# jwwangchn/BONAI

Measured on AMD Instinct MI355X. Metric: training img/s at 1024x1024 LOFT R50-FPN, higher is better.
Workload: dtype bf16; 1 GPU; LOFT R50-FPN + FOA, 8x1024x1024 synthetic tiles per GPU (BASELINE configs[1]), 80 gt/img, full train step (fwd+losses+bwd+allreduce+clip+SGD), random-init weights, RoI heads at the load of a trained RPN (first proposals = jittered gt boxes); global_batch=8, per_gpu_batch=8, parallelism=dp1, graph_features=False

## Files before the change

bonai_amd/csrc/elementwise.hip:

```cpp
#include "loft_common.h"
#include "../../include/loft_hip.h"
#include "conv_tap.h"

__device__ __forceinline__ void ld8(const bf16_t* p, float v[8]) {
    uint4 t = *reinterpret_cast<const uint4*>(p);
    unpack8_16(t, v);
}
__device__ __forceinline__ void st8(bf16_t* p, const float v[8]) {
    *reinterpret_cast<uint4*>(p) = pack8_16(v);
}

__device__ __forceinline__ void ld8(const float* p, float v[8]) { ld4(p, v); ld4(p + 4, v + 4); }
__device__ __forceinline__ void st8(float* p, const float v[8]) { st4(p, v); st4(p + 4, v + 4); }

static inline dim3 ew_grid(long nvec) {
    long b = (nvec + 255) / 256;
    if (b > 8192) b = 8192;
    if (b < 1) b = 1;
    return dim3((unsigned)b);
}

__global__ void relu_bwd_kernel(const bf16_t* __restrict__ g, const bf16_t* __restrict__ y, bf16_t* __restrict__ out,
                                long nvec) {
    for (long i = blockIdx.x * (long)blockDim.x + threadIdx.x; i < nvec; i += (long)gridDim.x * blockDim.x) {
// ... 1140 lines not shown
        const int r = i >> 5, cp = (i & 31) * 2;
        uint32_t v = 0;
        if (r0 + r < R && c0 + cp < Cc) v = *reinterpret_cast<const uint32_t*>(src + (long)(r0 + r) * Cc + c0 + cp);
        t[r][cp] = (bf16_t)(v & 0xffff);
        t[r][cp + 1] = (bf16_t)(v >> 16);
    }
    __syncthreads();
    for (int i = threadIdx.x; i < 64 * 32; i += 256) {
        const int c = i >> 5, rp = (i & 31) * 2;
        if (c0 + c < Cc && r0 + rp < R)
            *reinterpret_cast<uint32_t*>(dst + (long)(c0 + c) * R + r0 + rp) = (uint32_t)t[rp][c] | ((uint32_t)t[rp + 1][c] << 16);
    }
}
LOFT_EXPORT int loft_transpose_bf16(const void* src, void* dst, int R, int Cc, void* stream) {
    if (R <= 0 || Cc <= 0) return 0;
    if ((R & 1) || (Cc & 1)) return (int)hipErrorInvalidValue;
    hipLaunchKernelGGL(transpose_bf16_kernel, dim3(loft_cdiv(Cc, 64), loft_cdiv(R, 64)), dim3(256), 0, (hipStream_t)stream,
                       (const bf16_t*)src, (bf16_t*)dst, R, Cc);
    LOFT_LAUNCH_CHECK();
    return 0;
}

__global__ __launch_bounds__(256) void fold_unpack_bwd_kernel(const float* __restrict__ dwp, const float* __restrict__ db,
                                                              const float* __restrict__ w, const float* __restrict__ gamma,
                                                              const float* __restrict__ mean, const float* __restrict__ var,
                                                              float eps, int Cout, int Cin, int RS, float* __restrict__ dw,
                                                              float* __restrict__ dgamma, float* __restrict__ dbeta, int CoutP,
                                                              int CinP, int accumulate) {
    const int n = blockIdx.x;
    const float rs = gamma ? rsqrtf(var[n] + eps) : 1.f;
    const float scale = gamma ? gamma[n] * rs : 1.f;
    float acc = 0.f;
    const int per = Cin * RS;
    for (int j = threadIdx.x; j < per; j += blockDim.x) {
        const int c = j / RS, t = j - c * RS;
        const float g = dwp[((long)t * CoutP + n) * CinP + c];
        const long wi = (long)n * per + j;
        if (dw) dw[wi] = (accumulate ? dw[wi] : 0.f) + g * scale;
        if (gamma) acc += g * w[wi];
    }
    if (gamma) {
        for (int o = 32; o > 0; o >>= 1) acc += __shfl_down(acc, o, 64);
        __shared__ float part[4];
        if ((threadIdx.x & 63) == 0) part[threadIdx.x >> 6] = acc;
        __syncthreads();
        if (threadIdx.x == 0) {
            const float s = part[0] + part[1] + part[2] + part[3];
            const float dbn = db ? db[n] : 0.f;
            if (dgamma) dgamma[n] = (accumulate ? dgamma[n] : 0.f) + (s * rs - dbn * mean[n] * rs);
            if (dbeta) dbeta[n] = (accumulate ? dbeta[n] : 0.f) + dbn;
        }
    }
}
__global__ __launch_bounds__(256) void fold_unpack_bwd_multi_kernel(const long* __restrict__ desc, int njobs, int lds_floats) {
    const int lo = find_record(desc, njobs, (long)blockIdx.x);
    const long* d = desc + (long)lo * 16;
    const float* dwp = reinterpret_cast<const float*>(d[0]);
    const float* db = reinterpret_cast<const float*>(d[1]);
    const float* w = reinterpret_cast<const float*>(d[2]);
    const float* gamma = reinterpret_cast<const float*>(d[3]);
    const float* mean = reinterpret_cast<const float*>(d[4]);
    const float* var = reinterpret_cast<const float*>(d[5]);
    float* dw = reinterpret_cast<float*>(d[6]);
    float* dgamma = reinterpret_cast<float*>(d[7]);
    float* dbeta = reinterpret_cast<float*>(d[8]);
    const float eps = __int_as_float((int)(d[9] & 0xffffffffl));
    const int nsp = (int)(d[9] >> 32) > 1 ? (int)(d[9] >> 32) : 1;
    const int Cin = (int)d[11], CoutP = (int)d[13], CinP = (int)d[14];
    const bool nmajor = d[12] < 0;
    const int RS = (int)(nmajor ? -d[12] : d[12]);
    const int n = (int)(blockIdx.x - d[15]);
    const long sps = (long)RS * CoutP * CinP;
    auto ld1 = [&](const float* p) {
        float v = *p;
        int q = 1;
        for (; q + 3 < nsp; q += 4) {
            const float u0 = p[q * sps], u1 = p[(q + 1) * sps], u2 = p[(q + 2) * sps], u3 = p[(q + 3) * sps];
            v += (u0 + u1) + (u2 + u3);
        }
        for (; q < nsp; ++q) v += p[q * sps];
        return v;
    };
    auto ld4s = [&](const float* p) {
        float4 v = *reinterpret_cast<const float4*>(p);
        int q = 1;
        for (; q + 3 < nsp; q += 4) {
            const float4 u0 = *reinterpret_cast<const float4*>(p + q * sps), u1 = *reinterpret_cast<const float4*>(p + (q + 1) * sps);
            const float4 u2 = *reinterpret_cast<const float4*>(p + (q + 2) * sps), u3 = *reinterpret_cast<const float4*>(p + (q + 3) * sps);
            v.x += (u0.x + u1.x) + (u2.x + u3.x); v.y += (u0.y + u1.y) + (u2.y + u3.y);
            v.z += (u0.z + u1.z) + (u2.z + u3.z); v.w += (u0.w + u1.w) + (u2.w + u3.w);
        }
        for (; q < nsp; ++q) {
            const float4 u = *reinterpret_cast<const float4*>(p + q * sps);
            v.x += u.x; v.y += u.y; v.z += u.z; v.w += u.w;
        }
        return v;
    };
    const float rs = gamma ? rsqrtf(var[n] + eps) : 1.f;
    const float scale = gamma ? gamma[n] * rs : 1.f;
    float acc = 0.f;
    const int per = Cin * RS;
    if (nmajor) {
        extern __shared__ float urow[];
        const int CB = min(Cin, lds_floats / RS);
        const unsigned cb_mul = CB == 1 ? 0u : 0xFFFFFFFFu / (unsigned)CB + 1u;
        for (int cb0 = 0; cb0 < Cin; cb0 += CB) {
            const int cbn = min(CB, Cin - cb0), cnt = cbn * RS;
            const bool small = CB * RS < 65536 && cbn == CB;
            __syncthreads();
            for (int j = threadIdx.x; j < cnt; j += blockDim.x) {
                const int t = cbn == 1 ? j : (small ? (int)__umulhi((unsigned)j, cb_mul) : j / cbn), c = j - t * cbn;
                urow[c * RS + t] = ld1(dwp + (long)n * per + (long)t * CinP + cb0 + c);
            }
            __syncthreads();
            for (int j = threadIdx.x; j < cnt; j += blockDim.x) {
                const long wi = (long)n * per + (long)cb0 * RS + j;
                if (dw) dw[wi] += urow[j] * scale;
            }
        }
        if (threadIdx.x == 0 && dbeta && db) dbeta[n] += db[n];
        return;
    }
    if (RS > 1 && per <= lds_floats) {
        extern __shared__ float urow[];
        if ((Cin & 3) == 0 && (CinP & 3) == 0) {
            for (int j = threadIdx.x * 4; j < per; j += blockDim.x * 4) {
                const int t = j / Cin, c = j - t * Cin;
                const float4 v = ld4s(dwp + ((long)t * CoutP + n) * CinP + c);
                urow[c * RS + t] = v.x; urow[(c + 1) * RS + t] = v.y; urow[(c + 2) * RS + t] = v.z; urow[(c + 3) * RS + t] = v.w;
            }
            __syncthreads();
            for (int j = threadIdx.x * 4; j < per; j += blockDim.x * 4) {
                const float4 g = *reinterpret_cast<const float4*>(urow + j);
                const long wi = (long)n * per + j;
                if (dw) {
                    float4 o = *reinterpret_cast<float4*>(dw + wi);
                    o.x += g.x * scale; o.y += g.y * scale; o.z += g.z * scale; o.w += g.w * scale;
                    *reinterpret_cast<float4*>(dw + wi) = o;
                }
                if (gamma) {
                    const float4 ww = *reinterpret_cast<const float4*>(w + wi);
                    acc += g.x * ww.x + g.y * ww.y + g.z * ww.z + g.w * ww.w;
                }
            }
        } else {
            for (int j = threadIdx.x; j < per; j += blockDim.x) {
                const int t = j / Cin, c = j - t * Cin;
                urow[c * RS + t] = ld1(dwp + ((long)t * CoutP + n) * CinP + c);
            }
            __syncthreads();
            for (int j = threadIdx.x; j < per; j += blockDim.x) {
                const float g = urow[j];
                const long wi = (long)n * per + j;
                if (dw) dw[wi] += g * scale;
                if (gamma) acc += g * w[wi];
            }
        }
    } else if (RS == 1 && (Cin & 3) == 0 && (CinP & 3) == 0) {
        for (int j = threadIdx.x * 4; j < per; j += blockDim.x * 4) {
            const float4 g = ld4s(dwp + (long)n * CinP + j);
            const long wi = (long)n * per + j;
            if (dw) {
                float4 o = *reinterpret_cast<float4*>(dw + wi);
                o.x += g.x * scale; o.y += g.y * scale; o.z += g.z * scale; o.w += g.w * scale;
                *reinterpret_cast<float4*>(dw + wi) = o;
            }
            if (gamma) {
                const float4 ww = *reinterpret_cast<const float4*>(w + wi);
                acc += g.x * ww.x + g.y * ww.y + g.z * ww.z + g.w * ww.w;
            }
        }
    } else
    for (int j = threadIdx.x; j < per; j += blockDim.x) {
        const int c = j / RS, t = j - c * RS;
        const float g = ld1(dwp + ((long)t * CoutP + n) * CinP + c);
        const long wi = (long)n * per + j;
        if (dw) dw[wi] += g * scale;
        if (gamma) acc += g * w[wi];
    }
    if (gamma) {
        for (int o = 32; o > 0; o >>= 1) acc += __shfl_down(acc, o, 64);
        __shared__ float part[4];
        if ((threadIdx.x & 63) == 0) part[threadIdx.x >> 6] = acc;
        __syncthreads();
        if (threadIdx.x == 0) {
            const float s = part[0] + part[1] + part[2] + part[3];
            const float dbn = db ? db[n] : 0.f;
            if (dgamma) dgamma[n] += s * rs - dbn * mean[n] * rs;
            if (dbeta) dbeta[n] += dbn;
        }
    } else if (threadIdx.x == 0 && dbeta && db) {
        dbeta[n] += db[n];
    }
}
LOFT_EXPORT int loft_fold_unpack_bwd_multi(const int64_t* desc, int njobs, int64_t nblocks, int lds_floats, void* stream) {
    if (njobs <= 0 || nblocks <= 0) return 0;
    if (lds_floats < 0 || lds_floats > 16384) return (int)hipErrorInvalidValue;
    hipLaunchKernelGGL(fold_unpack_bwd_multi_kernel, dim3((unsigned)nblocks), dim3(256), (size_t)lds_floats * 4, (hipStream_t)stream,
                       (const long*)desc, njobs, lds_floats);
    LOFT_LAUNCH_CHECK();
    return 0;
}
LOFT_EXPORT int loft_fold_unpack_bwd(const float* dwp, const float* db, const float* w, const float* gamma, const float* mean,
                                     const float* var, float eps, int Cout, int Cin, int RS, float* dw, float* dgamma,
                                     float* dbeta, int CoutP, int CinP, int accumulate, void* stream) {
    if (Cout <= 0) return 0;
    if (CoutP < Cout || CinP < Cin) return (int)hipErrorInvalidValue;
    hipLaunchKernelGGL(fold_unpack_bwd_kernel, dim3(Cout), dim3(256), 0, (hipStream_t)stream, dwp, db, w, gamma, mean, var, eps,
                       Cout, Cin, RS, dw, dgamma, dbeta, CoutP, CinP, accumulate);
    LOFT_LAUNCH_CHECK();
    return 0;
}

template <typename T, int V> struct NhbIO;
template <> struct NhbIO<bf16_t, 4> {
    static __device__ __forceinline__ void ld(const bf16_t* p, float* v) { ld4(p, v); }
    static __device__ __forceinline__ void st(bf16_t* p, const float* v) { st4(p, v); }
};
template <> struct NhbIO<bf16_t, 8> {
    static __device__ __forceinline__ void ld(const bf16_t* p, float* v) { ld8(p, v); }
    static __device__ __forceinline__ void st(bf16_t* p, const float* v) { st8(p, v); }
};
template <> struct NhbIO<float, 4> {
    static __device__ __forceinline__ void ld(const float* p, float* v) {
        const float4 a = *reinterpret_cast<const float4*>(p);
        v[0] = a.x; v[1] = a.y; v[2] = a.z; v[3] = a.w;
    }
    static __device__ __forceinline__ void st(float* p, const float* v) { *reinterpret_cast<float4*>(p) = make_float4(v[0], v[1], v[2], v[3]); }
};

template <int NOUT, int V, typename XT = bf16_t>
__global__ __launch_bounds__(256) void narrow_head_bwd_kernel(const float* __restrict__ g, int gs, const XT* __restrict__ x,
                                                              const float* __restrict__ w, long M, int Cin, int relu_in,
                                                              XT* __restrict__ gx, float* __restrict__ dw,
                                                              float* __restrict__ db) {
    const int cg = Cin / V;
    const int ppi = 256 / cg > 0 ? 256 / cg : 1;
    const int tid = threadIdx.x;
    const int col = tid % cg, sub = tid / cg;
    const bool act = sub < ppi;
    const int c0 = col * V;
    float wr[NOUT][V], acc[NOUT][V], bacc[NOUT];
#pragma unroll
    for (int n = 0; n < NOUT; ++n) {
#pragma unroll
        for (int q = 0; q < V; ++q) { wr[n][q] = w[(long)n * Cin + c0 + q]; acc[n][q] = 0.f; }
        bacc[n] = 0.f;
    }
    if (act) {
        constexpr int UN = 4;
        const long step = ppi;
        const long per_blk = ((M + gridDim.x - 1) / gridDim.x + (long)ppi * UN - 1) / ((long)ppi * UN) * ((long)ppi * UN);
// ... 206 lines not shown
```

bonai_amd/debug.py:

```python
import contextlib
import os

SWITCHES = {
    'no_side_stream': 'mask / bbox branches, the RPN proposal chain and the backbone weight gradients all on the main stream '
                      '(the mode of bench.py\'s roofline instrumentation)',
    'no_bbox_side_stream': 'the bbox head on the main stream (the mask branch keeps its side stream)',
    'no_rpn_side_stream': 'the RPN proposal chain (sort, decode, NMS) on the main stream',
    'no_rpn_target_prefetch': 'RPN anchor assignment + sampling after the RPN convs on the main stream, not beside the backbone',
    'no_rpn_loss_stream': 'the RPN losses (and with them the sparse RPN backward) on the main stream',
    'no_wgrad_stream': 'backbone weight-gradient launches on the data-gradient stream',
    'unpack_stream': 'the batched weight-gradient unpack launches (descriptor upload + loft_fold_unpack_bwd_multi) on a stream of their '
                     'own instead of on the main stream between the data-gradient kernels (round 6: measured, not the default)',
    'no_prepack': 'BN fold + operand packing per conv per step instead of one launch per step (kernels.PrepackRegistry)',
    'no_unpack_queue': 'one loft_fold_unpack_bwd launch per conv instead of the batched unpack (kernels.UnpackQueue)',
    'no_grad_sink': 'gradients returned to autograd and accumulated by it, not deposited in the arena by the kernels',
    'no_leaf_sink': 'narrow heads and the sparse RPN backward return their parameter gradients to autograd (per-parameter accumulation '
                    'launches) instead of depositing them through the unpack queue (nn._queue_param_grads)',
    'no_head_fusion': 'narrow 1x1 heads (RPN objectness + deltas, mask logits) as launches of their own instead of in the producing '
                      'conv\'s epilogue (loft_conv_tap_bf16_head)',
    'no_grad_join': 'autograd sums the two data gradients of a backbone stage output (next stage + FPN lateral) with an elementwise add '
                    'instead of the residual block taking the lateral\'s deposit as its data-gradient residual (nn.JOIN)',
    'no_deconv_fusion': 'the mask head\'s 2x2 deconvolution as four parity launches instead of one launch whose four channel tiles are '
                        'the four taps (loft_deconv2x2_bf16: the input tile read once)',
    'no_zero_pool': 'torch.zeros / torch.empty per accumulation buffer instead of the step\'s pre-zeroed / scratch slabs',
    'no_feat_hub': 'autograd sums the RPN / RoI-extractor gradients of the FPN maps (no shared per-level gradient map)',
    'no_block_fusion': 'one autograd node per conv of a residual block instead of nn.res_block',
    'no_linear_fn': 'Linear layers through the generic conv node',
    'no_bneck_fusion': 'the frozen / inference 64-plane bottleneck as three (four) tap-conv launches instead of conv1 + the fused tail '
                       '(loft_bneck_tail_bf16: 3x3 + 1x1 expansion + shortcut + ReLU in one launch)',
    'no_pair_fusion': 'the last 1x1 of bottleneck k and the first 1x1 of bottleneck k+1 (layer2 / layer3) as two launches each way instead '
                      'of one (loft_bneck_pair_bf16: the block output is written once and not re-read as the next conv1\'s operand)',
    'wgrad_no_patch': 'the tap weight-gradient kernel for 64-channel high-resolution layers (no patch kernel)',
    'roi_fp32_bwd': 'RoIAlign backward into fp32 maps + a cast',
    'roi_sort': 'RoIAlign forward workgroups in (image, level, row strip) launch order for lists of >= 256 RoIs (loft_roi_order; '
                'measured neutral on the step, not shipped)',
    'no_roi_sort': 'list (sampling) order even where kernels.ROI_FWD_SORT_MIN asks for the launch order',
    'narrow_mfma_bwd': 'narrow (<= 8 output) heads backward as padded MFMA GEMMs',
}


class _Switches:
    __slots__ = tuple(SWITCHES)

    def __init__(self):
        for k in SWITCHES:
            setattr(self, k, bool(os.environ.get('LOFT_' + k.upper())))

    def active(self):
        return sorted(k for k in SWITCHES if getattr(self, k))

    @contextlib.contextmanager
    def override(self, **kw):
        prev = {k: getattr(self, k) for k in kw}
        try:
            for k, v in kw.items():
                setattr(self, k, bool(v))
            yield self
        finally:
            for k, v in prev.items():
                setattr(self, k, v)


DBG = _Switches()
```

bonai_amd/engine.py:

```python
import contextlib
import os

import torch
import torch.distributed as dist

from . import kernels as K
from . import nn as F2
from .debug import DBG
from .loss_scale import parse_loss_scale


class FlatArena:

    def __init__(self, model):
        self.params = [p for p in model.parameters() if p.requires_grad]
        dev = self.params[0].device
        order = list(reversed(self.params))
        self.offsets, off = {}, 0
        for p in order:
            self.offsets[id(p)] = off
            off += (p.numel() + 7) // 8 * 8
        self.numel = off
        self.data = torch.zeros(off, dtype=torch.float32, device=dev)
        self.grad = torch.zeros(off, dtype=torch.float32, device=dev)
# ... 208 lines not shown
    if it < warmup_iters:
        k = (1 - it / warmup_iters) * (1 - warmup_ratio)
        lr = lr * (1 - k)
    return lr


class Trainer:
    def __init__(self, model, lr=0.005, momentum=0.9, weight_decay=1e-4, max_norm=35.0, bucket_bytes=25 << 20,
                 loss_scale=1.0, graph_features=False, optimizer=None, paramwise_cfg=None):
        self.model = model
        self.graph_features = bool(graph_features)
        self._fgraphs = None
        self._unpack_stream = self._wgrad_stream = None
        self._steps_run = 0
        self.lr, self.mu, self.wd, self.max_norm = lr, momentum, weight_decay, (0.0 if max_norm is None else max_norm)
        self.optim = None
        if optimizer is not None or paramwise_cfg is not None:
            from .optim import build_spec
            if optimizer is None:
                optimizer = dict(type='SGD', lr=lr, momentum=momentum, weight_decay=weight_decay)
            self.optim = build_spec(optimizer, paramwise_cfg, model)
            h = self.optim.hyper
            self.lr, self.mu, self.wd = h['lr'], h.get('momentum', 0.0), h['weight_decay']
        mode, parsed = parse_loss_scale(loss_scale)
        self.loss_scale = parsed if mode == 'static' else None
        self.scaler = parsed if mode == 'dynamic' else None
        self.arena = FlatArena(model)
        self.reducer = BucketedAllReduce(self.arena, bucket_bytes)
        self._unpack_limit = int(os.environ.get('LOFT_UNPACK_LIMIT', '0')) or (24 if self.reducer.enabled else 48)
        self._unpack_note = self.reducer.note_queued if (self.reducer.enabled and os.environ.get('LOFT_NO_NOTE_FLUSH') != '1') else None
        self.world = dist.get_world_size() if self.reducer.enabled else 1
        self.gnorm_sq = torch.zeros(1, dtype=torch.float32, device=self.arena.data.device)
        self.scale_state = self._scale = None
        if self.scaler is not None:
            self.scale_state = K.loss_scale_state_pack(self.scaler['init_scale']).to(self.arena.data.device)
            self._scale = self.scale_state[K.LS_SCALE]
        self.seg_table = self.opt_state = self.exp_avg_sq = None
        self._plain_sgd = True
        if self.optim is not None:
            from .optim import arena_segments
            name = {id(p): n for n, p in model.named_parameters()}
            a = self.arena
            segs = arena_segments(self.optim, [(name[id(p)], a.offsets[id(p)], (p.numel() + 7) // 8 * 8) for p in a.order])
            if segs is not None:
                self.seg_table = K.SegmentTable(segs, a.numel, a.data.device)
            self._plain_sgd = self.optim.rule == 'SGD' and not self.optim.hyper['nesterov'] and segs is None
            if self.optim.rule == 'AdamW':
                self.exp_avg_sq = torch.zeros_like(a.momentum)
                if a.data.is_cuda:
                    self.opt_state = K.adamw_state_new(0, *self.optim.hyper['betas'], a.data.device)
        self.iter = 0
        self.prepack = K.PrepackRegistry()
        self._sink = self.reducer._sink if self.reducer.enabled else (lambda p: None)

    def _graph_step_setup(self, img):
        from .graphs import FeatureGraphs
        fg = self._fgraphs
        if fg is None:
            fg = self._fgraphs = FeatureGraphs(self)
        if fg.ready and fg.validate() is not None:
            import warnings
            warnings.warn(f'hipGraphs of backbone + neck dropped and recaptured: {fg.stale}', RuntimeWarning)
        if not fg.ready and fg.failed is None and self._steps_run >= 2 and self.prepack.order:
            self.reducer.capturing = True
            try:
                fg.capture(img)
            except Exception as e:
                import warnings
                fg.failed = f'{type(e).__name__}: {e}'
                warnings.warn(f'hipGraph capture of backbone + neck failed, the trainer stays on eager launches: {fg.failed}',
                              RuntimeWarning)
            finally:
                self.reducer.capturing = False
        if fg.ready:
            self.model.feat_provider = fg.provider

    def _config_optimizer_step(self, lr):
        a, o, c = self.arena, self.optim, self.scaler
        gscale = 1.0 / self.world if c is not None else 1.0 / (self.world * self.loss_scale)
        if o.rule == 'SGD':
            K.sgd_momentum_seg_(a.data, a.grad, a.momentum, self.gnorm_sq, self.max_norm, lr, self.mu, self.wd, grad_scale=gscale,
                                nesterov=o.hyper['nesterov'], table=self.seg_table, ls_state=self.scale_state)
        else:
            b1, b2 = o.hyper['betas']
            K.adamw_(a.data, a.grad, a.momentum, self.exp_avg_sq, self.gnorm_sq, self.max_norm, lr, b1, b2, o.hyper['eps'], self.wd,
                     self.opt_state, grad_scale=gscale, table=self.seg_table, ls_state=self.scale_state)
            K.adamw_state_advance_(self.opt_state, self.gnorm_sq, b1, b2, skip_nonfinite=c is not None)
        if c is not None:
            K.loss_scale_update_(self.scale_state, self.gnorm_sq, 1.0 / self.world, c['growth_factor'], c['backoff_factor'],
                                 c['growth_interval'], c['min_scale'], c['max_scale'])

    def _param_groups(self, base):
        named = list(self.model.named_parameters())
        if self.optim is None or not self.optim.paramwise:
            return [dict(base, params=list(range(len(named))))]
        groups = []
        for i, (n, p) in enumerate(named):
            lm, dm = self.optim.mult_of(n) if p.requires_grad else (1.0, 1.0)
            groups.append(dict(base, lr=base['lr'] * lm, weight_decay=base['weight_decay'] * dm, params=[i]))
        return groups

    def _adamw_state_dict(self):
        a, h = self.arena, self.optim.hyper
        idx = {id(p): i for i, p in enumerate(self.model.parameters())}
        state = {}
        if self.iter > 0:
# ... 61 lines not shown
                if id(p) in a.offsets:
                    todo.append((dst, a.offsets[id(p)], p.numel(), buf))
            if mine == 'AdamW' and id(p) in a.offsets and 'step' in st:
                steps.add(int(st['step']))
        if len(steps) > 1:
            raise RuntimeError(f'AdamW state with different step counts per parameter {sorted(steps)[:4]}: the arena keeps one')
        for dst, o, n, buf in todo:
            dst[o:o + n].copy_(buf.reshape(-1).to(dst.device))
        if mine == 'AdamW' and steps:
            self.opt_state.copy_(K.adamw_state_new(steps.pop(), *self.optim.hyper['betas'], self.opt_state.device))
        self.iter = int(sd.get('iter', self.iter))
        if 'sampler_calls' in sd:
            K._SAMPLE_CALLS[0] = int(sd['sampler_calls'])
        if self.scaler is not None and sd.get('loss_scaler') is not None:
            self.scale_state.copy_(K.loss_scale_state_pack(**sd['loss_scaler']))

    @contextlib.contextmanager
    def _step_scope(self):
        on = self.arena.data.is_cuda
        planes = dict(WEIGHT_PLANES=self.prepack.wplanes) if on and not DBG.no_prepack else {}
        F2.PAIR_G.clear()
        try:
            with F2.installed(JOIN={} if on and not DBG.no_grad_join else None, HUB=None, **planes):
                yield
        finally:
            F2.PAIR_G.clear()

    @contextlib.contextmanager
    def _forward_scope(self, data):
        on = self.arena.data.is_cuda
        prepack = dict(PREPACK=self.prepack) if on and not DBG.no_prepack else {}
        try:
            with F2.installed(HUB_ENABLED=on and not DBG.no_feat_hub, **prepack):
                if prepack:
                    self.prepack.run(self.iter)
                if self.graph_features and on and K.PROFILE is None and F2.PREPACK is not None and hasattr(self.model, 'extract_feat'):
                    self._graph_step_setup(data['img'])
                yield
        finally:
            if self.graph_features:
                self.model.feat_provider = None

    @contextlib.contextmanager
    def _backward_scope(self):
        on = self.arena.data.is_cuda
        sink = self._sink if on and not DBG.no_grad_sink else None
        queue = ustream = wstream = None
        try:
            if on and not DBG.no_zero_pool:
                K.zero_pool_begin(self.arena.data.device)
            if sink is not None and not DBG.no_unpack_queue:
                if DBG.unpack_stream and not DBG.no_side_stream:
                    ustream = self._unpack_stream = self._unpack_stream or torch.cuda.Stream()
                queue = K.UnpackQueue(limit=self._unpack_limit, note=self._unpack_note, stream=ustream)
                if not DBG.no_side_stream and not DBG.no_wgrad_stream:
                    wstream = self._wgrad_stream = self._wgrad_stream or torch.cuda.Stream()
            with F2.installed(GRAD_SINK=sink, UNPACK_Q=queue, WGRAD_STREAM=wstream):
                try:
                    yield
                finally:
                    if queue is not None:
                        queue.join()
        finally:
            K.zero_pool_end()

    def train_step(self, data, lr=None):
        self.arena.grad.zero_()
        self.arena.rebind_grads()
        self.reducer.begin()
        for p in self.arena.params:
            p._loft_pending = 0
            p._loft_sunk = False
        with self._step_scope():
            with self._forward_scope(data):
                out = self.model.train_step(data)
            with self._backward_scope():
                scale = self._scale if self.scaler is not None else self.loss_scale
                (out['loss'] if self.scaler is None and scale == 1.0 else out['loss'] * scale).backward()
                if F2.UNPACK_Q is not None:
                    F2.UNPACK_Q.flush()
        self.reducer.finish()
        self.gnorm_sq.zero_()
        K.sumsq_(self.arena.grad, self.gnorm_sq)
        if not self._plain_sgd:
            self._config_optimizer_step(self.lr if lr is None else lr)
        elif self.scaler is None:
            K.sgd_momentum_(self.arena.data, self.arena.grad, self.arena.momentum, self.gnorm_sq, self.max_norm,
                            self.lr if lr is None else lr, self.mu, self.wd, grad_scale=1.0 / (self.world * self.loss_scale))
        else:
            c = self.scaler
            K.sgd_momentum_scaled_(self.arena.data, self.arena.grad, self.arena.momentum, self.gnorm_sq, self.max_norm,
                                   self.lr if lr is None else lr, self.mu, self.wd, 1.0 / self.world, self.scale_state)
            K.loss_scale_update_(self.scale_state, self.gnorm_sq, 1.0 / self.world, c['growth_factor'], c['backoff_factor'],
                                 c['growth_interval'], c['min_scale'], c['max_scale'])
        self.iter += 1
        self._steps_run += 1
        return out
```

bonai_amd/kernels.py:

```python
import ctypes
import os

import numpy as np
import torch

from . import lib as L
from .debug import DBG as _DBG

c_int, c_int64, c_float, c_void_p = ctypes.c_int, ctypes.c_int64, ctypes.c_float, ctypes.c_void_p


def h2d(values, dtype, device):
    t = torch.from_numpy(values).to(dtype) if isinstance(values, np.ndarray) else torch.tensor(values, dtype=dtype)
    if torch.device(device).type != 'cuda':
        return t.to(device)
    if H2D_KEEP is not None:
        global _H2D_STREAM
        for _ in range(64):
            if _H2D_STREAM is None:
                _H2D_STREAM = torch.cuda.Stream()
            with torch.cuda.stream(_H2D_STREAM):
                if not torch.cuda.is_current_stream_capturing():
                    break
            _H2D_STREAM = None
# ... 2673 lines not shown

def random_sample(gt_inds, num, max_pos, mode='random'):
    lib = L.load()
    L.dev_check(gt_inds)
    gt_inds = gt_inds.contiguous()
    if gt_inds.dtype != torch.int64:
        raise L.LoftHipError(f'gt_inds must be int64, got {gt_inds.dtype}')
    B, N = gt_inds.shape
    P, Q = min(int(max_pos), N), min(int(num), N)
    dev = gt_inds.device
    pidx = torch.empty(B, P, dtype=torch.int64, device=dev)
    nidx = torch.empty(B, Q, dtype=torch.int64, device=dev)
    pval = torch.empty(B, P, dtype=torch.uint8, device=dev)
    nval = torch.empty(B, Q, dtype=torch.uint8, device=dev)
    _SAMPLE_CALLS[0] += 1
    seed = (torch.initial_seed() * 6364136223846793005 + _SAMPLE_CALLS[0] * 1442695040888963407) & 0xFFFFFFFFFFFFFFFF
    if B > 0 and N > 0:
        ws = torch.empty(B * ((N + 15) // 16 * 16), dtype=torch.uint8, device=dev)
        L.check(lib.loft_random_sample(L.ptr(gt_inds), B, N, int(num), int(max_pos), 0 if mode == 'first' else 1, seed, L.ptr(pidx),
                                       L.ptr(pval), L.ptr(nidx), L.ptr(nval), L.ptr(ws), L.stream()), 'loft_random_sample')
    return pidx, pval.view(torch.bool), nidx, nval.view(torch.bool)


def sampled_avg_factor(pos_valid, neg_valid):
    lib = L.load()
    L.dev_check(pos_valid, neg_valid)
    pv, nv = pos_valid.contiguous().view(torch.uint8), neg_valid.contiguous().view(torch.uint8)
    out = torch.empty(1, dtype=torch.float32, device=pv.device)
    L.check(lib.loft_sampled_avg_factor(L.ptr(pv), L.ptr(nv), int(pv.shape[0]), int(pv.shape[1]), int(nv.shape[1]), L.ptr(out),
                                        L.stream()), 'loft_sampled_avg_factor')
    return out


def narrow_head_bwd(g, x, w, relu_in=False, need_gx=True, need_dw=True, need_db=True):
    lib = L.load()
    L.dev_check(g, x, w)
    x = _nhwc(x)
    g = g.float().contiguous(memory_format=torch.channels_last)
    N, Cin, H, W = x.shape
    Cout = w.shape[0]
    w2 = w.reshape(Cout, Cin).float().contiguous()
    f32 = x.dtype == torch.float32
    gx = empty_nhwc(N, Cin, H, W, torch.float32 if f32 else L.act16(), x.device) if need_gx else None
    dw = pooled_zeros((Cout, Cin), x.device) if need_dw else None
    db = pooled_zeros((Cout,), x.device) if need_db else None
    fn = lib.loft_narrow_head_bwd_f32 if f32 else lib.loft_narrow_head_bwd
    L.check(fn(L.ptr(g), int(g.shape[1]), L.ptr(x), L.ptr(w2), N * H * W, Cin, Cout, int(relu_in),
               L.ptr(gx), L.ptr(dw), L.ptr(db), L.stream()), 'loft_narrow_head_bwd')
    return gx, dw, db


class UnpackQueue:

    def __init__(self, limit=48, note=None, stream=None):
        self.limit = limit
        self.note = note
        self.jobs, self.done = [], []
        self.main = torch.cuda.current_stream() if torch.cuda.is_available() else None
        self.main_raw = L.stream() if self.main is not None else None
        self.home = stream if stream is not None else self.main
        self.home_raw = self.home.cuda_stream if stream is not None else self.main_raw
        self.dedicated = stream is not None
        self.events = []
        self.main_jobs = False
        self.keep = []
        self._targets = set()

    def add(self, dwp, db, w, bn, eps, slots, on_done=(), flat_chw=None, nsplit=1, params=()):
        tgt = slots[0].data_ptr() if slots[0] is not None else None
        if tgt is not None:
            if tgt in self._targets:
                if os.environ.get('LOFT_DEBUG_TARGETS'):
                    print('unpack queue: slot used twice in one batch ->', tuple(w.shape), 'jobs pending', len(self.jobs), flush=True)
                self.flush()
            self._targets.add(tgt)
        self.jobs.append((dwp, db, w, bn, float(eps), slots, flat_chw, int(nsplit)))
        if self.home is not None:
            raw = L.stream()
            if raw == self.home_raw:
                pass
            elif self.dedicated and raw == self.main_raw:
                self.main_jobs = True
            else:
                ev = torch.cuda.Event()
                ev.record()
                self.events.append(ev)
                if not self.dedicated:
                    for t in (dwp, db):
                        if t is not None:
                            t.record_stream(self.home)
            if self.dedicated:
                self.keep.append((dwp, db))
        self.done.extend(on_done)
        if len(self.jobs) >= self.limit or (self.note is not None and self.note(params)):
            self.flush()

    def join(self, stream=None):
        if self.dedicated:
            (stream or self.main).wait_stream(self.home)
        self.keep = []

    def flush(self):
        if self.home is not None and L.stream() != self.home_raw:
            if self.main_jobs:
                ev = torch.cuda.Event()
                ev.record(self.main)
                self.events.append(ev)
                self.main_jobs = False
            with torch.cuda.stream(self.home):
                return self.flush()
        for ev in self.events:
            self.home.wait_event(ev)
        self.events = []
        if self.jobs:
            import struct
            rows, blk = [], 0
            p = lambda t: 0 if t is None else t.data_ptr()
            for dwp, db, w, bn, eps, (dw, dg, dbeta), flat, nsplit in self.jobs:
                if flat is not None:
                    Cout, Cin, RS = w.shape[0], flat[0], -(flat[1] * flat[2])
                    coutp, cinp = Cout, Cin
                else:
                    Cout, Cin = w.shape[0], w.shape[1]
                    RS = w.shape[2] * w.shape[3] if w.dim() == 4 else 1
                    coutp, cinp = dwp.shape[-2], dwp.shape[-1]
                g, _, m, v = bn if bn is not None else (None, None, None, None)
                rows.append([p(dwp), p(db), p(w), p(g), p(m), p(v), p(dw), p(dg), p(dbeta),
                             (struct.unpack('<I', struct.pack('<f', eps))[0]) | (nsplit << 32), Cout, Cin, RS, coutp, cinp, blk])
                blk += Cout
            desc = h2d(rows, torch.int64, self.jobs[0][2].device)
            lds = max([min(r[11], 64) * abs(r[12]) if r[12] < 0 else r[11] * r[12] for r in rows
                       if r[12] < 0 or (r[12] > 1 and r[11] * r[12] <= 16384)], default=0)
            if lds > 16384:
                raise L.LoftHipError(f'fold_unpack_bwd_multi: a record needs {lds} floats of LDS')
            L.check(L.load().loft_fold_unpack_bwd_multi(L.ptr(desc), len(rows), blk, int(lds), L.stream()), 'loft_fold_unpack_bwd_multi')
            self.jobs = []
            self._targets = set()
        done, self.done = self.done, []
        for f in done:
            f()


def fold_unpack_bwd(dwp, db, w, bn=None, eps=1e-5, need_dw=True, out=None):
    lib = L.load()
    w = w.contiguous()
    Cout, Cin, R, S = w.shape
    dev = w.device
    g = m = v = dg = dbeta = None
    if out is not None:
        dw, dg, dbeta = out
        if bn is not None:
            g, _, m, v = [t.contiguous() for t in bn]
    else:
        dw = torch.empty_like(w) if need_dw else None
        if bn is not None:
            g, _, m, v = [t.contiguous() for t in bn]
            dg = torch.empty(Cout, dtype=torch.float32, device=dev)
            dbeta = torch.empty(Cout, dtype=torch.float32, device=dev)
    L.check(lib.loft_fold_unpack_bwd(L.ptr(dwp), L.ptr(db), L.ptr(w), L.ptr(g), L.ptr(m), L.ptr(v), eps, Cout, Cin,
                                     R * S, L.ptr(dw), L.ptr(dg), L.ptr(dbeta), dwp.shape[-2], dwp.shape[-1], int(out is not None),
                                     L.stream()),
            'loft_fold_unpack_bwd')
    return dw, dg, dbeta
```

include/loft_hip.h:

```cpp
#ifndef LOFT_HIP_H
#define LOFT_HIP_H
#include <stdint.h>

#ifdef __cplusplus
extern "C" {
#endif

#define LOFT_F32 0
#define LOFT_BF16 1
#define LOFT_F16 2
int loft_act16_dtype(void);

int loft_roi_align_fwd(const void* const* feats_host, const int* H_host, const int* W_host, const float* scales_host,
                       int num_levels, int finest_scale, int C, int dtype, const float* rois, int K, int P,
                       int n_rot, void* out, void* stream);
int loft_roi_align_bwd(void* const* grad_feats_host, const int* H_host, const int* W_host, const float* scales_host,
                       int num_levels, int finest_scale, int C, int dtype, const float* rois, int K, int P,
                       int n_rot, const void* grad_out, int B, int accumulate, int rois_sorted, void* workspace,
                       int grad_dtype, void* stream);
#define LOFT_ROI_AUTO 0
#define LOFT_ROI_FWD_SAMPLE 1
#define LOFT_ROI_FWD_SEP4 2
#define LOFT_ROI_BWD_VALU 1
#define LOFT_ROI_BWD_PIPE 2
// ... 338 lines not shown
                      float* rois, void* stream);

int loft_rpn_gather_rows(void* const* level_ptrs, const int* H, const int* W, int n_levels, const int* rows, int nsel, int C,
                         int K, void* out, void* stream);
int loft_rpn_scatter_add_rows(void* const* level_ptrs, const int* H, const int* W, int n_levels, const int* rows, int nsel,
                              int C, int K, const void* src, void* stream);

int loft_rpn_sparse_prep(const float* g, const int64_t* slot, int nsel, int A, int P, int C, const float* w_cls, const float* w_reg,
                         const float* w_conv, void* g_rows, void* w_headT, void* wd, void* stream);

int loft_fuse_sum_relu(const void* const* terms, const int* shifts, int n_terms, void* out, int dtype, int B, int H, int W,
                       int C, int relu, void* stream);
int loft_blocksum_masked(const void* g, const void* y, void* out, int dtype, int B, int Hc, int Wc, int C, int shift,
                         void* stream);
int loft_bilinear_up_slot(const void* src, void* dst, int dtype, int B, int h, int w, int C, int shift, int Ctot, int coff,
                          int backward, void* stream);
int loft_avgpool(const void* src, void* dst, int dtype, int B, int Ho, int Wo, int C, int shift, int backward, int accumulate,
                 void* stream);
int loft_stem3x3s2_bn_relu(const float* img, const float* w, const float* scale, const float* shift, void* out, int dtype,
                           int B, int H, int W, void* stream);
int loft_stem3x3s2_wgrad(const float* img, const void* g, const void* y, float* dwp, float* db, int dtype, int B, int H, int W,
                         void* stream);
int loft_stem7x7_pool_wgrad(const float* img, const void* y, const void* gp, float* dwp, float* db, int dtype, int B, int H,
                            int W, void* stream);

int loft_mdcn_sample_fwd(const void* x, const float* offmask, void* col, int dtype, int B, int IH, int IW, int C, int OH,
                         int OW, int kh, int kw, int stride, int pad, int dil, int deform_groups, int offmask_stride,
                         void* stream);
int loft_mdcn_sample_bwd(const void* x, const float* offmask, const void* dcol, float* dx, float* doffmask, int dtype, int B,
                         int IH, int IW, int C, int OH, int OW, int kh, int kw, int stride, int pad, int dil,
                         int deform_groups, int offmask_stride, void* workspace, void* stream);
int64_t loft_mdcn_bwd_workspace_bytes(int B, int C, int OH, int OW, int kh, int kw, int stride, int dil, int deform_groups,
                                      int offmask_stride);
#define LOFT_MDCN_AUTO 0
#define LOFT_MDCN_BWD_GENERIC 1
#define LOFT_MDCN_BWD_TILE 2
#define LOFT_MDCN_BWD_BIN 3
#define LOFT_MDCN_VARIANT(family, count) ((family) | ((count) << 8))
int loft_mdcn_sample_bwd_v(const void* x, const float* offmask, const void* dcol, float* dx, float* doffmask, int dtype, int B,
                           int IH, int IW, int C, int OH, int OW, int kh, int kw, int stride, int pad, int dil,
                           int deform_groups, int offmask_stride, void* workspace, int variant, void* stream);
int64_t loft_mdcn_bwd_workspace_bytes_v(int B, int C, int OH, int OW, int kh, int kw, int stride, int dil, int deform_groups,
                                        int offmask_stride, int variant);
int loft_mdcn_bwd_form(int B, int IH, int IW, int C, int OH, int OW, int kh, int kw, int stride, int pad, int dil,
                       int deform_groups, int offmask_stride, int dtype, int variant);

int loft_fold_pack(const float* w, const float* conv_bias, const float* gamma, const float* beta, const float* mean,
                   const float* var, float eps, int Cout, int Cin, int RS, void* wp_fwd, void* wp_dgrad, float* bias_out,
                   int pack_f32, int CoutP, int CinP, void* stream);
int loft_fold_pack_multi(const int64_t* desc, int n, int64_t nchunks, void* stream);
int loft_fold_f32_multi(const int64_t* desc, int n, int64_t nblocks, void* stream);
int loft_split_planes_f32_multi(const int64_t* desc, int n, int64_t nblocks, void* stream);
int loft_fold_unpack_bwd_multi(const int64_t* desc, int njobs, int64_t nblocks, int lds_floats, void* stream);
int loft_transpose_bf16(const void* src, void* dst, int R, int Cc, void* stream);
int loft_fold_unpack_bwd(const float* dwp, const float* db, const float* w, const float* gamma, const float* mean,
                         const float* var, float eps, int Cout, int Cin, int RS, float* dw, float* dgamma, float* dbeta,
                         int CoutP, int CinP, int accumulate, void* stream);

int loft_narrow_head_bwd(const float* g, int g_stride, const void* x, const float* w, int64_t M, int Cin, int Cout,
                         int relu_in, void* gx, float* dw, float* db, void* stream);
int loft_narrow_head_bwd_f32(const float* g, int g_stride, const float* x, const float* w, int64_t M, int Cin, int Cout,
                             int relu_in, float* gx, float* dw, float* db, void* stream);

int64_t loft_random_sample_workspace_bytes(int B, int N);
int loft_random_sample(const int64_t* gt_inds, int B, int N, int num, int max_pos, int mode, uint64_t seed,
                       int64_t* pos_idx, uint8_t* pos_valid, int64_t* neg_idx, uint8_t* neg_valid, void* workspace, void* stream);

int loft_rpn_sample_gather(const void* const* heads, const int* H, const int* W, const int64_t* lvl_off, int num_levels,
                           int B, int Cp, int A, const float* anchors, const float* gts, int Kmax,
                           const int64_t* gt_inds, int64_t N, const int64_t* pos_idx, const uint8_t* pos_valid, int P,
                           const int64_t* neg_idx, const uint8_t* neg_valid, int Q, const float* means_host,
                           const float* stds_host, float* vals, int32_t* rows, int64_t* slot, float* tgt,
                           int64_t* label, float* weight, void* stream);

int loft_sampled_avg_factor(const uint8_t* pos_valid, const uint8_t* neg_valid, int B, int P, int Q, float* out, void* stream);

int loft_fused_loss(int mode, const float* pred, const void* target, const float* weight, int64_t n, int C,
                    const float* avg_factor, float count, float scale, float beta, float* grad, float* partial,
                    uint32_t* counter, float* loss_out, void* stream);
int loft_fused_loss_v2(int mode, const float* pred, int64_t d1, int64_t d2, int64_t s0, int64_t s1, int64_t s2, const void* target,
                       int target_kind, const void* weight, int weight_kind, int64_t wdiv, int64_t n, int C, const float* avg_factor,
                       float count, float scale, float beta, float* grad, float* partial, uint32_t* counter, float* loss_out,
                       int want_acc, void* stream);

int loft_roi_sample_offsets(const uint8_t* pos_valid, const uint8_t* neg_valid, int B, int P, int Q, int32_t* tab, void* stream);
int loft_roi_sample_targets(const float* cand, int Ncand, const int64_t* gt_inds, const float* gts,
                            const int64_t* gt_labels, int Kmax, const int64_t* pos_idx, const int64_t* neg_idx, int P,
                            int Q, int B, const int32_t* npos_dev, const int32_t* nneg_dev, const int32_t* roi_off_dev,
                            const int32_t* pos_off_dev, int num_classes, const float* means_host, const float* stds_host,
                            float* rois, int64_t* labels, float* label_weights, float* bbox_targets, float* bbox_weights,
                            float* pos_rois, int64_t* pos_img, int64_t* pos_gt, int64_t* pos_row, void* stream);

int loft_coco_box_iou(const double* dt, const double* gt, const uint8_t* iscrowd, int D, int G, double* out, void* stream);
int loft_coco_mask_iou(const int* inter, const int* area_p, const int* area_g, const uint8_t* iscrowd, int D, int G, double* out,
                       void* stream);
#define LOFT_COCO_MAX_GT 4096
#define LOFT_COCO_MAX_THRS 16
#define LOFT_COCO_MAX_RECS 128
#define LOFT_COCO_TOO_MANY_GT (-2)
int loft_coco_match(const double* ious, const int64_t* iou_off, const int64_t* det_off, const int64_t* gt_off,
                    const double* det_area, const double* gt_area, const uint8_t* gt_crowd, const double* thrs,
                    const double* area_rng, int S, int64_t total_det, int max_gt, int T, int A, int32_t* gt_match,
                    uint8_t* det_ign, uint64_t* bits, int32_t* npig, void* stream);
int loft_coco_accumulate(const uint64_t* bits, const int32_t* rank, const int32_t* perm, int64_t N, const int64_t* npig,
                         const int32_t* max_dets, const double* rec_thrs, int T, int A, int M, int R, double* precision,
                         double* recall, void* stream);
// ... 6 lines not shown
```

Before: 236.1 img/s.

## Store first weight-gradient deposit instead of zero-filling the whole gradient arena

Adds a templated unpack kernel variant that overwrites a gradient slot on its first deposit of the step instead of read-modify-write accumulation. The engine learns over one step which arena slots are always first-written by the unpack queue, then zero-fills only the remaining ranges on later steps. This removes a full-arena memset and the read half of each first accumulation. In exchange it adds host-side bookkeeping, extra queue flushes when side slots collide, and a fallback path that re-zeroes slots a step fails to reach.

After: 236.1 img/s (median of 2 runs). No clear change (+0.0%).

```diff
diff --git a/bonai_amd/csrc/elementwise.hip b/bonai_amd/csrc/elementwise.hip
--- a/bonai_amd/csrc/elementwise.hip
+++ b/bonai_amd/csrc/elementwise.hip
@@ -1216,6 +1216,7 @@
         }
     }
 }
+template <bool FIRST>
 __global__ __launch_bounds__(256) void fold_unpack_bwd_multi_kernel(const long* __restrict__ desc, int njobs, int lds_floats) {
     const int lo = find_record(desc, njobs, (long)blockIdx.x);
     const long* d = desc + (long)lo * 16;
@@ -1229,7 +1230,10 @@
     float* dgamma = reinterpret_cast<float*>(d[7]);
     float* dbeta = reinterpret_cast<float*>(d[8]);
     const float eps = __int_as_float((int)(d[9] & 0xffffffffl));
-    const int nsp = (int)(d[9] >> 32) > 1 ? (int)(d[9] >> 32) : 1;
+    const int nsp_w = FIRST ? (int)((d[9] >> 32) & 0xffff) : (int)(d[9] >> 32);
+    const int nsp = nsp_w > 1 ? nsp_w : 1;
+    const int first = FIRST ? (int)((d[9] >> 48) & 7) : 0;
+    const bool st_w = first & 1, st_g = first & 2, st_b = first & 4;
     const int Cin = (int)d[11], CoutP = (int)d[13], CinP = (int)d[14];
     const bool nmajor = d[12] < 0;
     const int RS = (int)(nmajor ? -d[12] : d[12]);
@@ -1279,10 +1283,10 @@
             __syncthreads();
             for (int j = threadIdx.x; j < cnt; j += blockDim.x) {
                 const long wi = (long)n * per + (long)cb0 * RS + j;
-                if (dw) dw[wi] += urow[j] * scale;
-            }
-        }
-        if (threadIdx.x == 0 && dbeta && db) dbeta[n] += db[n];
+                if (dw) dw[wi] = (st_w ? 0.f : dw[wi]) + urow[j] * scale;
+            }
+        }
+        if (threadIdx.x == 0 && dbeta && db) dbeta[n] = (st_b ? 0.f : dbeta[n]) + db[n];
         return;
     }
     if (RS > 1 && per <= lds_floats) {
@@ -1298,7 +1302,7 @@
                 const float4 g = *reinterpret_cast<const float4*>(urow + j);
                 const long wi = (long)n * per + j;
                 if (dw) {
-                    float4 o = *reinterpret_cast<float4*>(dw + wi);
+                    float4 o = st_w ? make_float4(0.f, 0.f, 0.f, 0.f) : *reinterpret_cast<float4*>(dw + wi);
                     o.x += g.x * scale; o.y += g.y * scale; o.z += g.z * scale; o.w += g.w * scale;
                     *reinterpret_cast<float4*>(dw + wi) = o;
                 }
@@ -1316,7 +1320,7 @@
             for (int j = threadIdx.x; j < per; j += blockDim.x) {
                 const float g = urow[j];
                 const long wi = (long)n * per + j;
-                if (dw) dw[wi] += g * scale;
+                if (dw) dw[wi] = (st_w ? 0.f : dw[wi]) + g * scale;
                 if (gamma) acc += g * w[wi];
             }
         }
@@ -1325,7 +1329,7 @@
             const float4 g = ld4s(dwp + (long)n * CinP + j);
             const long wi = (long)n * per + j;
             if (dw) {
-                float4 o = *reinterpret_cast<float4*>(dw + wi);
+                float4 o = st_w ? make_float4(0.f, 0.f, 0.f, 0.f) : *reinterpret_cast<float4*>(dw + wi);
                 o.x += g.x * scale; o.y += g.y * scale; o.z += g.z * scale; o.w += g.w * scale;
                 *reinterpret_cast<float4*>(dw + wi) = o;
             }
@@ -1339,7 +1343,7 @@
         const int c = j / RS, t = j - c * RS;
         const float g = ld1(dwp + ((long)t * CoutP + n) * CinP + c);
         const long wi = (long)n * per + j;
-        if (dw) dw[wi] += g * scale;
+        if (dw) dw[wi] = (st_w ? 0.f : dw[wi]) + g * scale;
         if (gamma) acc += g * w[wi];
     }
     if (gamma) {
@@ -1350,18 +1354,26 @@
         if (threadIdx.x == 0) {
             const float s = part[0] + part[1] + part[2] + part[3];
             const float dbn = db ? db[n] : 0.f;
-            if (dgamma) dgamma[n] += s * rs - dbn * mean[n] * rs;
-            if (dbeta) dbeta[n] += dbn;
+            if (dgamma) dgamma[n] = (st_g ? 0.f : dgamma[n]) + (s * rs - dbn * mean[n] * rs);
+            if (dbeta) dbeta[n] = (st_b ? 0.f : dbeta[n]) + dbn;
         }
     } else if (threadIdx.x == 0 && dbeta && db) {
-        dbeta[n] += db[n];
+        dbeta[n] = (st_b ? 0.f : dbeta[n]) + db[n];
     }
 }
 LOFT_EXPORT int loft_fold_unpack_bwd_multi(const int64_t* desc, int njobs, int64_t nblocks, int lds_floats, void* stream) {
     if (njobs <= 0 || nblocks <= 0) return 0;
     if (lds_floats < 0 || lds_floats > 16384) return (int)hipErrorInvalidValue;
-    hipLaunchKernelGGL(fold_unpack_bwd_multi_kernel, dim3((unsigned)nblocks), dim3(256), (size_t)lds_floats * 4, (hipStream_t)stream,
-                       (const long*)desc, njobs, lds_floats);
+    hipLaunchKernelGGL(fold_unpack_bwd_multi_kernel<false>, dim3((unsigned)nblocks), dim3(256), (size_t)lds_floats * 4,
+                       (hipStream_t)stream, (const long*)desc, njobs, lds_floats);
+    LOFT_LAUNCH_CHECK();
+    return 0;
+}
+LOFT_EXPORT int loft_fold_unpack_bwd_multi_first(const int64_t* desc, int njobs, int64_t nblocks, int lds_floats, void* stream) {
+    if (njobs <= 0 || nblocks <= 0) return 0;
+    if (lds_floats < 0 || lds_floats > 16384) return (int)hipErrorInvalidValue;
+    hipLaunchKernelGGL(fold_unpack_bwd_multi_kernel<true>, dim3((unsigned)nblocks), dim3(256), (size_t)lds_floats * 4,
+                       (hipStream_t)stream, (const long*)desc, njobs, lds_floats);
     LOFT_LAUNCH_CHECK();
     return 0;
 }
diff --git a/bonai_amd/debug.py b/bonai_amd/debug.py
--- a/bonai_amd/debug.py
+++ b/bonai_amd/debug.py
@@ -22,6 +22,9 @@
                     'instead of the residual block taking the lateral\'s deposit as its data-gradient residual (nn.JOIN)',
     'no_deconv_fusion': 'the mask head\'s 2x2 deconvolution as four parity launches instead of one launch whose four channel tiles are '
                         'the four taps (loft_deconv2x2_bf16: the input tile read once)',
+    'no_store_first': 'the whole gradient arena zero-filled every step and every weight-gradient deposit accumulated into it, instead '
+                      'of the unpack storing a slot\'s first deposit of the step (loft_fold_unpack_bwd_multi_first) and the fill '
+                      'covering only the slots no such deposit reaches',
     'no_zero_pool': 'torch.zeros / torch.empty per accumulation buffer instead of the step\'s pre-zeroed / scratch slabs',
     'no_feat_hub': 'autograd sums the RPN / RoI-extractor gradients of the FPN maps (no shared per-level gradient map)',
     'no_block_fusion': 'one autograd node per conv of a residual block instead of nn.res_block',
diff --git a/bonai_amd/engine.py b/bonai_amd/engine.py
--- a/bonai_amd/engine.py
+++ b/bonai_amd/engine.py
@@ -284,6 +284,70 @@
         self.iter = 0
         self.prepack = K.PrepackRegistry()
         self._sink = self.reducer._sink if self.reducer.enabled else (lambda p: None)
+        self._store_plan = self._store_first = None
+        self._store_mode, self._store_hooks, self._store_fed, self._queue_seen = None, [], set(), None
+
+    _STORE_MERGE_GAP = 1 << 16
+
+    def _store_key(self):
+        return (tuple(DBG.active()), str(K.L.act16()), self.arena.grad.data_ptr())
+
+    def _store_first_begin(self):
+        a = self.arena
+        ok = (a.data.is_cuda and not self.graph_features and not DBG.no_store_first and not DBG.no_grad_sink
+              and not DBG.no_unpack_queue)
+        plan = self._store_plan
+        if ok and plan is not None and plan[0] == self._store_key():
+            for lo, hi in plan[2]:
+                a.grad[lo:hi].zero_()
+            a.rebind_grads()
+            self._store_mode = 'apply'
+            return plan[1]
+        self._store_plan = None
+        a.grad.zero_()
+        a.rebind_grads()
+        self._store_mode = 'learn' if ok else None
+        if ok:
+            fed = self._store_fed = set()
+
+            def hook(p):
+                if not getattr(p, '_loft_sunk', False):
+                    fed.add(id(p))
+            self._store_hooks = [p.register_post_accumulate_grad_hook(hook) for p in a.order]
+        return None
+
+    def _store_first_abort(self):
+        for h in self._store_hooks:
+            h.remove()
+        self._store_hooks, self._store_mode, self._store_plan, self._queue_seen = [], None, None, None
+
+    def _store_first_end(self):
+        a, mode, seen = self.arena, self._store_mode, self._queue_seen
+        for h in self._store_hooks:
+            h.remove()
+        self._store_hooks, self._store_mode, self._queue_seen = [], None, None
+        base = a.grad.data_ptr()
+        if mode == 'apply':
+            missing = self._store_plan[1] - (seen or set())
+            if missing:
+                for p in a.order:
+                    if base + 4 * a.offsets[id(p)] in missing:
+                        p.grad.zero_()
+                self._store_plan = None
+        elif mode == 'learn' and seen:
+            ptrs, ranges = set(), []
+            for p in a.order:
+                o = a.offsets[id(p)]
+                if base + 4 * o in seen and id(p) not in self._store_fed and getattr(p, '_loft_sunk', False):
+                    ptrs.add(base + 4 * o)
+                    continue
+                hi = o + (p.numel() + 7) // 8 * 8
+                if ranges and o - ranges[-1][1] < self._STORE_MERGE_GAP:
+                    ranges[-1][1] = hi
+                else:
+                    ranges.append([o, hi])
+            if ptrs:
+                self._store_plan = (self._store_key(), ptrs, [tuple(r) for r in ranges])
 
     def _graph_step_setup(self, img):
         from .graphs import FeatureGraphs
@@ -451,7 +515,8 @@
             if sink is not None and not DBG.no_unpack_queue:
                 if DBG.unpack_stream and not DBG.no_side_stream:
                     ustream = self._unpack_stream = self._unpack_stream or torch.cuda.Stream()
-                queue = K.UnpackQueue(limit=self._unpack_limit, note=self._unpack_note, stream=ustream)
+                queue = K.UnpackQueue(limit=self._unpack_limit, note=self._unpack_note, stream=ustream, first=self._store_first)
+                self._queue_seen = queue.seen
                 if not DBG.no_side_stream and not DBG.no_wgrad_stream:
                     wstream = self._wgrad_stream = self._wgrad_stream or torch.cuda.Stream()
             with F2.installed(GRAD_SINK=sink, UNPACK_Q=queue, WGRAD_STREAM=wstream):
@@ -464,20 +529,24 @@
             K.zero_pool_end()
 
     def train_step(self, data, lr=None):
-        self.arena.grad.zero_()
-        self.arena.rebind_grads()
+        self._store_first = self._store_first_begin()
         self.reducer.begin()
         for p in self.arena.params:
             p._loft_pending = 0
             p._loft_sunk = False
-        with self._step_scope():
-            with self._forward_scope(data):
-                out = self.model.train_step(data)
-            with self._backward_scope():
-                scale = self._scale if self.scaler is not None else self.loss_scale
-                (out['loss'] if self.scaler is None and scale == 1.0 else out['loss'] * scale).backward()
-                if F2.UNPACK_Q is not None:
-                    F2.UNPACK_Q.flush()
+        try:
+            with self._step_scope():
+                with self._forward_scope(data):
+                    out = self.model.train_step(data)
+                with self._backward_scope():
+                    scale = self._scale if self.scaler is not None else self.loss_scale
+                    (out['loss'] if self.scaler is None and scale == 1.0 else out['loss'] * scale).backward()
+                    if F2.UNPACK_Q is not None:
+                        F2.UNPACK_Q.flush()
+        except BaseException:
+            self._store_first_abort()
+            raise
+        self._store_first_end()
         self.reducer.finish()
         self.gnorm_sq.zero_()
         K.sumsq_(self.arena.grad, self.gnorm_sq)
diff --git a/bonai_amd/kernels.py b/bonai_amd/kernels.py
--- a/bonai_amd/kernels.py
+++ b/bonai_amd/kernels.py
@@ -2749,8 +2749,10 @@
 
 class UnpackQueue:
 
-    def __init__(self, limit=48, note=None, stream=None):
+    def __init__(self, limit=48, note=None, stream=None, first=None):
         self.limit = limit
+        self.first = first
+        self.seen = set()
         self.note = note
         self.jobs, self.done = [], []
         self.main = torch.cuda.current_stream() if torch.cuda.is_available() else None
@@ -2771,7 +2773,20 @@
                     print('unpack queue: slot used twice in one batch ->', tuple(w.shape), 'jobs pending', len(self.jobs), flush=True)
                 self.flush()
             self._targets.add(tgt)
-        self.jobs.append((dwp, db, w, bn, float(eps), slots, flat_chw, int(nsplit)))
+        flags = 0
+        ptrs = [None if t is None else t.data_ptr() for t in slots]
+        if self.first is not None:
+            side = [q for q in ptrs[1:] if q is not None]
+            if any(q in self._targets for q in side):
+                self.flush()
+                if tgt is not None:
+                    self._targets.add(tgt)
+            self._targets.update(side)
+            for bit, q in enumerate(ptrs):
+                if q is not None and q in self.first and q not in self.seen:
+                    flags |= 1 << bit
+        self.seen.update(q for q in ptrs if q is not None)
+        self.jobs.append((dwp, db, w, bn, float(eps), slots, flat_chw, int(nsplit) | flags << 16))
         if self.home is not None:
             raw = L.stream()
             if raw == self.home_raw:
@@ -2824,13 +2839,19 @@
                 g, _, m, v = bn if bn is not None else (None, None, None, None)
                 rows.append([p(dwp), p(db), p(w), p(g), p(m), p(v), p(dw), p(dg), p(dbeta),
                              (struct.unpack('<I', struct.pack('<f', eps))[0]) | (nsplit << 32), Cout, Cin, RS, coutp, cinp, blk])
+                if self.first is not None and (nsplit & 0xffff) >= 0x8000:
+                    raise L.LoftHipError(f'fold_unpack_bwd_multi_first: {nsplit & 0xffff} split-K slots do not fit the descriptor')
                 blk += Cout
             desc = h2d(rows, torch.int64, self.jobs[0][2].device)
             lds = max([min(r[11], 64) * abs(r[12]) if r[12] < 0 else r[11] * r[12] for r in rows
                        if r[12] < 0 or (r[12] > 1 and r[11] * r[12] <= 16384)], default=0)
             if lds > 16384:
                 raise L.LoftHipError(f'fold_unpack_bwd_multi: a record needs {lds} floats of LDS')
-            L.check(L.load().loft_fold_unpack_bwd_multi(L.ptr(desc), len(rows), blk, int(lds), L.stream()), 'loft_fold_unpack_bwd_multi')
+            if self.first is None:
+                L.check(L.load().loft_fold_unpack_bwd_multi(L.ptr(desc), len(rows), blk, int(lds), L.stream()), 'loft_fold_unpack_bwd_multi')
+            else:
+                L.check(L.load().loft_fold_unpack_bwd_multi_first(L.ptr(desc), len(rows), blk, int(lds), L.stream()),
+                        'loft_fold_unpack_bwd_multi_first')
             self.jobs = []
             self._targets = set()
         done, self.done = self.done, []
diff --git a/include/loft_hip.h b/include/loft_hip.h
--- a/include/loft_hip.h
+++ b/include/loft_hip.h
@@ -414,6 +414,7 @@
 int loft_fold_f32_multi(const int64_t* desc, int n, int64_t nblocks, void* stream);
 int loft_split_planes_f32_multi(const int64_t* desc, int n, int64_t nblocks, void* stream);
 int loft_fold_unpack_bwd_multi(const int64_t* desc, int njobs, int64_t nblocks, int lds_floats, void* stream);
+int loft_fold_unpack_bwd_multi_first(const int64_t* desc, int njobs, int64_t nblocks, int lds_floats, void* stream);
 int loft_transpose_bf16(const void* src, void* dst, int R, int Cc, void* stream);
 int loft_fold_unpack_bwd(const float* dwp, const float* db, const float* w, const float* gamma, const float* mean,
                          const float* var, float eps, int Cout, int Cin, int RS, float* dw, float* dgamma, float* dbeta,
```
